# pasqal-io/Pulser

Measured on NVIDIA B200. Metric: time-steps/s (1 ns sampling intervals of the Sequence evolved per second), higher is better.
Workload: dtype f64 (complex128)

## Files before the change

pulser_b200/csrc/kernels.cuh:

```cuda
#pragma once
#include <cuda_runtime.h>
#include <stdint.h>

namespace pb200 {

struct c2 { double x, y; };

__host__ __device__ inline c2 cmul(c2 a, c2 b) { return {a.x * b.x - a.y * b.y, a.x * b.y + a.y * b.x}; }
__host__ __device__ inline c2 cadd(c2 a, c2 b) { return {a.x + b.x, a.y + b.y}; }

struct PassGeom {
    int n_bits;
    int lo_bits;
    int hi_shift;
    int hi_bits;
    uint32_t tile_flip_mask;
    unsigned long long extra_mask;
    int first_pass;
};

struct StageCoef {
    c2 c_psi, c_b2, c_g;
};

// ... 573 lines not shown
    for (unsigned long long em = g.extra_mask; em; em &= em - 1) {
        const int p = __ffsll((long long)em) - 1;
        const double sg = (((base >> p) & 1) == to_bit) ? 1.0 : -1.0;
        double2 raw[R];
#pragma unroll
        for (int r = 0; r < R; ++r) raw[r] = __ldg(reinterpret_cast<const double2*>(vsrc + (idx_of(r) ^ (1LL << p))));
#pragma unroll
        for (int r = 0; r < R; ++r) {
            pr[r] += raw[r].x; pi[r] += raw[r].y;
            if (!REAL_G) { qr[r] = fma(sg, raw[r].x, qr[r]); qi[r] = fma(sg, raw[r].y, qi[r]); }
        }
    }
    mbar_wait(&mbar, 0);
    const int jstart = __ffs(g.tile_flip_mask) - 1;
    c2 v[R];
#pragma unroll
    for (int r = 0; r < R; ++r) v[r] = tile[tid + r * NT];
    rb_tile_gather<true, REAL_G, TBITS, RB>(g, tile, nullptr, tid, to_bit, jstart, false, v, pr, pi, qr, qi);
#pragma unroll
    for (int r = 0; r < R; ++r) {
        double dx = a.u.g.x * pr[r], dy = a.u.g.x * pi[r];
        if (!REAL_G) { dx = fma(-a.u.g.y, qi[r], dx); dy = fma(a.u.g.y, qr[r], dy); }
        const c2 gv = {fma(dg[r], v[r].x, dx), fma(dg[r], v[r].y, dy)};
        const c2 res = cadd(part[r], cmul(a.coef.c_g, gv));
        st_c2(a.out + voff + idx_of(r), res);
        v[r] = res;
    }
    if (a.w_out) {
#pragma unroll
        for (int r = 0; r < R; ++r) {
            rtile[tid + r * NT] = v[r];
            pr[r] = 0.0; pi[r] = 0.0; qr[r] = 0.0; qi[r] = 0.0;
        }
        __syncthreads();
        rb_tile_gather<true, REAL_G, TBITS, RB>(g, rtile, nullptr, tid, to_bit, jstart, false, v, pr, pi, qr, qi);
#pragma unroll
        for (int r = 0; r < R; ++r) {
            const long long ix = idx_of(r);
            st_c2(a.w_out + voff + ix, c2{pr[r], pi[r]});
            if (!REAL_G) st_c2(a.w_out + a.w_plane + voff + ix, c2{qr[r], qi[r]});
        }
    }
}

#define PB200_TAYLOR_PMAX 8
struct TaylorArgs {
    const c2* v;
    c2* out;
    c2* g_out;
    c2* acc;
    const double* dint;
    long long dint_stride;
    long long D;
    PassGeom geo;
    c2 unit;
    const double* table;
    int to_bit, from_is_one;
    double th0, gam0, om0, m0;
    c2 scale;
    int nh;
    const c2* hchi[PB200_TAYLOR_PMAX];
    const c2* hg[PB200_TAYLOR_PMAX];
    double hth[PB200_TAYLOR_PMAX], hgam[PB200_TAYLOR_PMAX], hom[PB200_TAYLOR_PMAX], hm[PB200_TAYLOR_PMAX];
    int acc_read;
    int acc_add_v;
    int acc_on;
    c2 acc_mul;
};

template <int R>
__device__ __forceinline__ void taylor_epilogue(const TaylorArgs& a, const long long (&idx)[R], const c2 (&v)[R],
                                                const double (&gx)[R], const double (&gy)[R], const double (&off)[R],
                                                long long voff, const double* __restrict__ dsrc) {
    constexpr int H = (R >= 4) ? R / 2 : R;
    const int nb = a.geo.n_bits;
#pragma unroll
    for (int h0 = 0; h0 < R; h0 += H) {
        double sx[H], sy[H], cn[H];
        {
            double dv[H];
#pragma unroll
            for (int r = 0; r < H; ++r) dv[r] = dsrc ? __ldcs(dsrc + idx[h0 + r]) : 0.0;
#pragma unroll
            for (int r = 0; r < H; ++r) {
                const int ones = __popcll((unsigned long long)idx[h0 + r]);
                cn[r] = (double)(a.from_is_one ? ones : (nb - ones));
                const double diag = fma(-a.th0, cn[r], fma(-a.m0, off[h0 + r], dv[r] - a.gam0));
                sx[r] = fma(diag, v[h0 + r].x, a.om0 * gx[h0 + r]);
                sy[r] = fma(diag, v[h0 + r].y, a.om0 * gy[h0 + r]);
            }
        }
        for (int j = 0; j < a.nh; ++j) {
            if (a.hchi[j]) {
                c2 c[H];
#pragma unroll
                for (int r = 0; r < H; ++r) c[r] = ld_own(a.hchi[j] + voff + idx[h0 + r]);
#pragma unroll
                for (int r = 0; r < H; ++r) {
                    const double d = -fma(a.hth[j], cn[r], fma(a.hm[j], off[h0 + r], a.hgam[j]));
                    sx[r] = fma(d, c[r].x, sx[r]); sy[r] = fma(d, c[r].y, sy[r]);
                }
            }
            if (a.hg[j]) {
                c2 c[H];
#pragma unroll
                for (int r = 0; r < H; ++r) c[r] = ld_own(a.hg[j] + voff + idx[h0 + r]);
#pragma unroll
                for (int r = 0; r < H; ++r) { sx[r] = fma(a.hom[j], c[r].x, sx[r]); sy[r] = fma(a.hom[j], c[r].y, sy[r]); }
            }
        }
        c2 res[H];
#pragma unroll
        for (int r = 0; r < H; ++r) {
            res[r] = {a.scale.x * sx[r] - a.scale.y * sy[r], a.scale.x * sy[r] + a.scale.y * sx[r]};
            st_c2(a.out + voff + idx[h0 + r], res[r]);
            if (a.g_out) st_c2(a.g_out + voff + idx[h0 + r], c2{gx[h0 + r], gy[h0 + r]});
        }
        if (a.acc_on) {
            c2 ac[H];
#pragma unroll
            for (int r = 0; r < H; ++r) ac[r] = a.acc_read ? ld_own(a.acc + voff + idx[h0 + r]) : c2{0.0, 0.0};
#pragma unroll
            for (int r = 0; r < H; ++r) {
                c2 s = cadd(ac[r], res[r]);
                if (a.acc_add_v) s = cadd(s, v[h0 + r]);
                st_c2(a.acc + voff + idx[h0 + r], cmul(a.acc_mul, s));
            }
        }
    }
}

template <bool UNIFORM, bool REAL_G, int TBITS, int RB>
__global__ void __launch_bounds__(1 << (TBITS - RB), (65536 / ((1 << (TBITS - RB)) * (RB >= 3 ? 128 : 64))))
stage_d2_taylor_kernel(const __grid_constant__ TaylorArgs a) {
    constexpr int R = 1 << RB;
    constexpr int NT = 1 << (TBITS - RB);
    constexpr int TSIZE = 1 << TBITS;
    extern __shared__ __align__(128) unsigned char smem_raw[];
    c2* tile = reinterpret_cast<c2*>(smem_raw);
    __shared__ __align__(8) uint64_t mbar;
    const PassGeom& g = a.geo;
    const int tid = threadIdx.x;
    const long long traj = UNIFORM ? 0 : (long long)blockIdx.y;
    const long long voff = traj * a.D;
    const long long base = tile_base_of(g, blockIdx.x);
    const c2* vsrc = a.v + voff;

    if (tid == 0) mbar_init(&mbar, 1);
    __syncthreads();
    pdl_wait();
    pdl_launch_dependents();
    if (tid == 0) mbar_arrive_expect_tx(&mbar, (uint32_t)TSIZE * 16u);
    {
        const int rows = 1 << g.hi_bits;
        const uint32_t row_bytes = (uint32_t)(16u << g.lo_bits);
        for (int r = tid; r < rows; r += NT)
            tma_load_1d(tile + ((size_t)r << g.lo_bits), vsrc + base + ((long long)r << g.hi_shift), row_bytes, &mbar);
    }
    double* tab = reinterpret_cast<double*>(tile + TSIZE);
    if (!UNIFORM) {
        const int stride = d2_table_stride(g.n_bits);
        const double* src = a.table + traj * stride;
        for (int i = tid; i < stride; i += NT) tab[i] = src[i];
        __syncthreads();
    }
    const long long lomask = (1LL << g.lo_bits) - 1;
    const int to_bit = a.to_bit;
    c2 v[R];
    double pr[R], pi[R], qr[R], qi[R];
    long long idx[R];
#pragma unroll
    for (int r = 0; r < R; ++r) {
        const int t = tid + r * NT;
        idx[r] = base | (t & lomask) | ((long long)(t >> g.lo_bits) << g.hi_shift);
        pr[r] = 0.0; pi[r] = 0.0; qr[r] = 0.0; qi[r] = 0.0;
    }
    for (unsigned long long m = g.extra_mask; m; m &= m - 1) {
        const int p = __ffsll((long long)m) - 1;
        const int bit = (int)((base >> p) & 1);
        const double sg = (bit == to_bit) ? 1.0 : -1.0;
        double gx = 0.0, gy = 0.0;
        if (!UNIFORM) { gx = tab[2 * p]; gy = (bit == to_bit) ? tab[2 * p + 1] : -tab[2 * p + 1]; }
        double2 raw[R];
#pragma unroll
        for (int r = 0; r < R; ++r) raw[r] = __ldg(reinterpret_cast<const double2*>(vsrc + (idx[r] ^ (1LL << p))));
#pragma unroll
        for (int r = 0; r < R; ++r) {
            if (UNIFORM) {
                pr[r] += raw[r].x; pi[r] += raw[r].y;
                if (!REAL_G) { qr[r] = fma(sg, raw[r].x, qr[r]); qi[r] = fma(sg, raw[r].y, qi[r]); }
            } else {
                pr[r] = fma(gx, raw[r].x, pr[r]); pr[r] = fma(-gy, raw[r].y, pr[r]);
                pi[r] = fma(gx, raw[r].y, pi[r]); pi[r] = fma(gy, raw[r].x, pi[r]);
            }
        }
    }
    mbar_wait(&mbar, 0);
#pragma unroll
    for (int r = 0; r < R; ++r) v[r] = tile[tid + r * NT];
    rb_tile_gather<UNIFORM, REAL_G, TBITS, RB>(g, tile, tab, tid, to_bit, 0, false, v, pr, pi, qr, qi);
    double off[R];
    if (UNIFORM) {
#pragma unroll
        for (int r = 0; r < R; ++r) {
            const double dx = a.unit.x * pr[r], dy = a.unit.x * pi[r];
            if (!REAL_G) { pr[r] = fma(-a.unit.y, qi[r], dx); pi[r] = fma(a.unit.y, qr[r], dy); }
            else { pr[r] = dx; pi[r] = dy; }
            off[r] = 0.0;
        }
    } else {
        const int nb = g.n_bits;
        const long long fixed = base | (tid & lomask) | ((long long)(tid >> g.lo_bits) << g.hi_shift);
        double common = 0.0;
        for (int p = 0; p < nb; ++p) {
            const int bit = (int)((fixed >> p) & 1);
            common += (bit == a.from_is_one) ? tab[2 * nb + p] : 0.0;
        }
#pragma unroll
        for (int r = 0; r < R; ++r) {
            double acc = common;
#pragma unroll
            for (int q = 0; q < RB; ++q) {
                const int j = TBITS - RB + q;
                const int p = (j < g.lo_bits) ? j : (j - g.lo_bits + g.hi_shift);
                const double th = tab[2 * nb + p];
                const int bit = (r >> q) & 1;
                acc += ((bit == a.from_is_one) ? th : 0.0) - ((0 == a.from_is_one) ? th : 0.0);
            }
            off[r] = acc;
        }
    }
    taylor_epilogue<R>(a, idx, v, pr, pi, off, voff, a.dint ? a.dint + traj * a.dint_stride : nullptr);
}

__global__ void __launch_bounds__(256) stage_d2_taylor_small_kernel(const __grid_constant__ TaylorArgs a) {
    const long long s = (long long)blockIdx.x * blockDim.x + threadIdx.x;
    if (s >= a.D) return;
    const int nb = a.geo.n_bits;
    const long long traj = blockIdx.y;
    const long long voff = traj * a.D;
    const double* tab = a.table ? a.table + traj * d2_table_stride(nb) : nullptr;
    double gxs = 0.0, gys = 0.0, offv = 0.0;
    if (tab) {
        for (int p = 0; p < nb; ++p) {
            const double2 raw = __ldg(reinterpret_cast<const double2*>(a.v + voff + (s ^ (1LL << p))));
            const int bit = (int)((s >> p) & 1);
            const double gx = tab[2 * p], gy = (bit == a.to_bit) ? tab[2 * p + 1] : -tab[2 * p + 1];
            gxs = fma(gx, raw.x, gxs); gxs = fma(-gy, raw.y, gxs);
            gys = fma(gx, raw.y, gys); gys = fma(gy, raw.x, gys);
            offv += (bit == a.from_is_one) ? tab[2 * nb + p] : 0.0;
        }
    } else {
        double pr = 0.0, pi = 0.0, qr = 0.0, qi = 0.0;
        for (int p = 0; p < nb; ++p) {
            const double2 raw = __ldg(reinterpret_cast<const double2*>(a.v + voff + (s ^ (1LL << p))));
            const double sg = ((int)((s >> p) & 1) == a.to_bit) ? 1.0 : -1.0;
            pr += raw.x; pi += raw.y; qr = fma(sg, raw.x, qr); qi = fma(sg, raw.y, qi);
        }
        gxs = fma(-a.unit.y, qi, a.unit.x * pr);
        gys = fma(a.unit.y, qr, a.unit.x * pi);
    }
    const long long idx[1] = {s};
    const double2 own = __ldg(reinterpret_cast<const double2*>(a.v + voff + s));
    const c2 v[1] = {{own.x, own.y}};
    const double gx[1] = {gxs}, gy[1] = {gys}, off[1] = {offv};
    taylor_epilogue<1>(a, idx, v, gx, gy, off, voff, a.dint ? a.dint + traj * a.dint_stride : nullptr);
}

__host__ __device__ inline int gen_table_stride(int n, int n_drives) { return n_drives * 3 * n + 3; }

#define PB200_TILED_MAX_HIGH 40
#define PB200_MAX_DRIVES_K 3
struct GenArgs {
    const c2* v; const c2* psi; const c2* b2; c2* out;
    const double* dint; long long dint_stride; long long D;
    int n, dim, n_drives;
    int to[3], from[3];
    StageCoef coef;
    const double* table;
    const double* beta_dev;
    const double* xy; long long xy_stride; int xy_u, xy_d;
    unsigned long long slm_mask; const double* dint2;
    double* dot_acc;
    LanczosFuse lz;
};

__global__ void __launch_bounds__(256) stage_generic_kernel(GenArgs a) {
    extern __shared__ __align__(16) unsigned char smem_raw[];
    double* tab = reinterpret_cast<double*>(smem_raw);
    const int stride = gen_table_stride(a.n, a.n_drives);
    const long long traj = blockIdx.y;
    for (int i = threadIdx.x; i < stride; i += blockDim.x) tab[i] = a.table[traj * stride + i];
    __syncthreads();
    double* xys = tab + stride;
    if (a.xy) {
        const double wx = tab[stride - 2], wxc = tab[stride - 3];
        for (int i = threadIdx.x; i < a.n * a.n; i += blockDim.x) {
            const int qi = i / a.n, qj = i - qi * a.n;
            const bool touched = ((a.slm_mask >> qi) | (a.slm_mask >> qj)) & 1ULL;
            xys[i] = a.xy[traj * a.xy_stride + i] * (touched ? wxc : wx);
        }
        __syncthreads();
    }
    const double w = tab[stride - 2], gamma = tab[stride - 1];
    const long long voff = traj * a.D;
    for (long long idx = blockIdx.x * (long long)blockDim.x + threadIdx.x; idx < a.D;
         idx += (long long)gridDim.x * blockDim.x) {
        const c2 vo = a.v[voff + idx];
        double diag = -gamma;
        if (a.dint) diag = fma(w, a.dint[traj * a.dint_stride + idx], diag);
        if (a.dint2) diag = fma(tab[stride - 3], a.dint2[traj * a.dint_stride + idx], diag);
        double rr = 0.0, ri = 0.0;
        long long rem = idx, st = 1;
        for (int k = a.n - 1; k >= 0; --k) {
            const int digit = (int)(rem % a.dim);
            rem /= a.dim;
            for (int q = 0; q < a.n_drives; ++q) {
                const double* gq = tab + q * 3 * a.n;
                if (digit == a.to[q]) {
// ... 659 lines not shown
```

pulser_b200/csrc/plan.cu:

```cuda
#include <cuda_runtime.h>

#include <algorithm>
#include <map>
#include <mutex>
#include <unordered_map>
#include <cmath>
#include <complex>
#include <cstdarg>
#include <cstdio>
#include <cstdlib>
#include <cstring>
#include <stdexcept>
#include <string>
#include <vector>

#include "../../include/pulser_b200.h"
#include "kernels.cuh"
#include "spline.hpp"
#include <cub/device/device_scan.cuh>
#include <nvtx3/nvToolsExt.h>
#include <random>

namespace pb200 {

// ... 51 lines not shown
    std::multimap<size_t, void*> free_list[PB200_MAX_DEVICES];
    std::unordered_map<void*, size_t> size_of;
    size_t held[PB200_MAX_DEVICES] = {0};
};
static DevicePool& pool() { static DevicePool* p = new DevicePool(); return *p; }

static void* pool_alloc(int dev, size_t bytes) {
    if (bytes == 0) bytes = 16;
    bytes = (bytes + 255) & ~(size_t)255;
    DevicePool& pl = pool();
    if (dev >= 0 && dev < PB200_MAX_DEVICES) {
        std::lock_guard<std::mutex> lk(pl.mu);
        auto it = pl.free_list[dev].lower_bound(bytes);
        if (it != pl.free_list[dev].end() && it->first <= bytes + bytes / 4) {
            void* p = it->second;
            pl.held[dev] -= it->first;
            pl.free_list[dev].erase(it);
            return p;
        }
    }
    void* p = nullptr;
    cudaError_t e = cudaMalloc(&p, bytes);
    if (e != cudaSuccess) {
        cudaGetLastError();
        {
            std::lock_guard<std::mutex> lk(pl.mu);
            if (dev >= 0 && dev < PB200_MAX_DEVICES) {
                for (auto& kv : pl.free_list[dev]) { pl.size_of.erase(kv.second); cudaFree(kv.second); }
                pl.free_list[dev].clear(); pl.held[dev] = 0;
            }
        }
        CUDA_CHECK(cudaMalloc(&p, bytes));
    }
    std::lock_guard<std::mutex> lk(pl.mu);
    pl.size_of[p] = bytes;
    return p;
}

static void pool_free(int dev, void* p) {
    if (!p) return;
    DevicePool& pl = pool();
    static const size_t cap = (size_t)std::max(0, env_int("PB200_POOL_MIB", 16384)) << 20;
    {
        std::lock_guard<std::mutex> lk(pl.mu);
        auto it = pl.size_of.find(p);
        if (it != pl.size_of.end() && dev >= 0 && dev < PB200_MAX_DEVICES && pl.held[dev] + it->second <= cap) {
            pl.free_list[dev].emplace(it->second, p);
            pl.held[dev] += it->second;
            return;
        }
        if (it != pl.size_of.end()) pl.size_of.erase(it);
    }
    cudaFree(p);
}

static int device_setup(int dev) {
    static std::mutex mu;
    static int sm_count[PB200_MAX_DEVICES] = {0};
    std::lock_guard<std::mutex> lk(mu);
    if (dev >= 0 && dev < PB200_MAX_DEVICES && sm_count[dev] > 0) return sm_count[dev];
    int sms = 0;
    CUDA_CHECK(cudaDeviceGetAttribute(&sms, cudaDevAttrMultiProcessorCount, dev));
    const int max_smem = (1 << 13) * 16 + 1024;
    CUDA_CHECK(cudaFuncSetAttribute(stage_d2_kernel<true, true>, cudaFuncAttributeMaxDynamicSharedMemorySize, max_smem));
    CUDA_CHECK(cudaFuncSetAttribute(stage_d2_kernel<true, false>, cudaFuncAttributeMaxDynamicSharedMemorySize, max_smem));
    CUDA_CHECK(cudaFuncSetAttribute(stage_d2_kernel<false, false>, cudaFuncAttributeMaxDynamicSharedMemorySize, max_smem));
#define PB200_RB_ATTR(TB, RB)                                                                                                            \
    CUDA_CHECK(cudaFuncSetAttribute(stage_d2_rb_kernel<true, true, TB, RB>, cudaFuncAttributeMaxDynamicSharedMemorySize, max_smem));   \
    CUDA_CHECK(cudaFuncSetAttribute(stage_d2_rb_kernel<true, false, TB, RB>, cudaFuncAttributeMaxDynamicSharedMemorySize, max_smem));  \
    CUDA_CHECK(cudaFuncSetAttribute(stage_d2_rb_kernel<false, false, TB, RB>, cudaFuncAttributeMaxDynamicSharedMemorySize, max_smem));
    PB200_RB_ATTR(11, 2) PB200_RB_ATTR(11, 3) PB200_RB_ATTR(12, 2) PB200_RB_ATTR(12, 3)
#undef PB200_RB_ATTR
    CUDA_CHECK(cudaFuncSetAttribute(stage_d2_taylor_kernel<true, true, 11, 3>, cudaFuncAttributeMaxDynamicSharedMemorySize, 2048 * 16 + 256));
    CUDA_CHECK(cudaFuncSetAttribute(stage_d2_taylor_kernel<true, false, 11, 3>, cudaFuncAttributeMaxDynamicSharedMemorySize, 2048 * 16 + 256));
    CUDA_CHECK(cudaFuncSetAttribute(stage_d2_taylor_kernel<false, false, 11, 3>, cudaFuncAttributeMaxDynamicSharedMemorySize, 2048 * 16 + 2048));
    CUDA_CHECK(cudaFuncSetAttribute(stage_d2_fwd_kernel<true, 11, 3>, cudaFuncAttributeMaxDynamicSharedMemorySize, 2 * 2048 * 16 + 256));
    CUDA_CHECK(cudaFuncSetAttribute(stage_d2_fwd_kernel<false, 11, 3>, cudaFuncAttributeMaxDynamicSharedMemorySize, 2 * 2048 * 16 + 256));
    if (dev >= 0 && dev < PB200_MAX_DEVICES) sm_count[dev] = sms;
    return sms;
}

struct DriveTables {
    std::vector<PiecewiseCubic<cplx>> coef;
    std::vector<PiecewiseCubic<double>> det;
    std::vector<double> coef_scale, det_scale;
};

struct Plan {
    pb200_plan_desc desc;
    std::vector<double> times;
    int n = 0, dim = 0, B = 1;
    long long D = 0;
    int n_drives = 0;
    cudaStream_t stream = nullptr;
    bool own_stream = false;
    c2* buf[3] = {nullptr, nullptr, nullptr};
    c2* aux[6] = {nullptr, nullptr, nullptr, nullptr, nullptr, nullptr};
    int cur = 0;
    double* dint = nullptr;
    bool dint_shared = true;
    bool has_interaction = false;
    double* d_table = nullptr;
    size_t d_table_cap = 0;
    double* d_scratch = nullptr;
    std::vector<std::vector<DriveTables>> tabs;
    std::vector<std::vector<bool>> tabs_set;
    std::vector<double> dmin_cnt, dmax_cnt;
    std::vector<double> dmin_traj, dmax_traj;
    bool state_set = false;
    int tile_bits = 12;
    int max_extra = 3;
    int sm_count = 148;
    bool force_v1 = false;
    int reg_bits = 3;
    bool use_dual = true;
    std::vector<std::vector<cplx>> diss_gen;
    c2* kry = nullptr; int kry_cap = 0;
    double* d_kry = nullptr;
    int m_last = 8;
    bool use_krylov = false;
    long long kry_iters = 0;
    bool has_diss = false;
    std::vector<std::vector<cplx>> jump_ops;
    std::vector<std::vector<double>> jump_ldl;
    std::vector<std::vector<cplx>> jump_ldl_full;
    bool jump_diag = true;
    bool has_collapse = false;
    double* d_xy = nullptr; bool xy_shared = true; bool has_xy = false; int xy_u = 0, xy_d = 1;
// ... 1047 lines not shown
            for (int dgt = 0; P.jump_diag && dgt < P.dim; ++dgt) {
                CUDA_CHECK(cudaMemsetAsync(d_occ, 0, sizeof(double) * P.n, P.stream));
                const long long nb = std::min<long long>((P.D + 255) / 256, (long long)P.sm_count * 4);
                occupation_kernel<<<(unsigned)std::max<long long>(nb, 1), 256, sizeof(double) * P.n, P.stream>>>(
                    psi, d_occ, P.D, P.n, P.dim, dgt);
                CUDA_CHECK(cudaMemcpyAsync(occ.data() + (size_t)dgt * P.n, d_occ, sizeof(double) * P.n, cudaMemcpyDeviceToHost, P.stream));
            }
            CUDA_CHECK(cudaStreamSynchronize(P.stream));
            for (size_t op = 0; P.jump_diag && op < P.jump_ops.size(); ++op)
                for (int k = 0; k < P.n; ++k) {
                    double wv = 0.0;
                    for (int dgt = 0; dgt < P.dim; ++dgt) wv += P.jump_ldl[op][dgt] * occ[(size_t)dgt * P.n + k];
                    wts[op * P.n + k] = wv; tot += wv;
                }
            if (tot <= 0.0) { P.thresholds[tr] = uni(P.rng); continue; }
            double x = uni(P.rng) * tot; size_t sel = 0;
            for (; sel + 1 < wts.size(); ++sel) { x -= wts[sel]; if (x <= 0.0) break; }
            const size_t op = sel / P.n; const int k = (int)(sel % P.n);
            QuditOp qo{};
            for (int q = 0; q < P.dim * P.dim; ++q) qo.m[q] = {P.jump_ops[op][q].real(), P.jump_ops[op][q].imag()};
            long long stq = 1;
            for (int q = 0; q < P.n - 1 - k; ++q) stq *= P.dim;
            const double scale = 1.0 / std::sqrt(std::max(wts[sel], 1e-300));
            const long long nb = std::min<long long>((P.D / P.dim + 255) / 256, (long long)P.sm_count * 8);
            qudit_op_kernel<<<(unsigned)std::max<long long>(nb, 1), 256, 0, P.stream>>>(psi, P.D, P.dim, stq, scale, qo);
            CUDA_CHECK(cudaGetLastError());
            st.n_launches += 1 + P.dim;
            P.thresholds[tr] = uni(P.rng);
            P.jump_count[tr] += 1;
        }
        t = b;
    }
    norms2();
    for (int tr = 0; tr < P.B; ++tr) {
        if (norms[tr] <= 0.0) continue;
        const double sc = 1.0 / std::sqrt(norms[tr]);
        scale_kernel<<<(unsigned)std::max<long long>(blocks, 1), 256, 0, P.stream>>>(P.buf[P.cur] + (size_t)tr * P.D, P.D, sc);
        P.thresholds[tr] /= norms[tr];
        P.thresholds[tr] = std::min(P.thresholds[tr], 1.0);
    }
    CUDA_CHECK(cudaGetLastError());
    pool_free(P.desc.device, d_occ);
    CUDA_CHECK(cudaEventRecord(ev1, P.stream));
    CUDA_CHECK(cudaEventSynchronize(ev1));
    float ms = 0.f;
    CUDA_CHECK(cudaEventElapsedTime(&ms, ev0, ev1));
    st.gpu_ms = ms; st.integrator = 1; st.mean_step_samples = K;
    if (stats) *stats = st;
}

static thread_local const char* g_taylor_why = "";
static bool taylor_prepare(Plan& P);
static bool taylor_worthwhile(Plan& P, double gtol);
static bool taylor_geometry(const Plan& P, const std::vector<PassGeom>& passes, bool& use_rb);
static void propagate_taylor(Plan& P, double t_start, double t_stop, const pb200_run_opts* o, pb200_run_stats* stats);

static void propagate(Plan& P, double t_start, double t_stop, const pb200_run_opts* o, pb200_run_stats* stats) {
    if (!P.state_set) fail(PB200_ERR_STATE, "pb200_propagate: no state set (call pb200_state_set first)");
    for (int tr = 0; tr < P.B; ++tr)
        for (int q = 0; q < P.n_drives; ++q)
            if (!P.tabs_set[tr][q]) fail(PB200_ERR_STATE, "pb200_propagate: drive %d of trajectory %d not set", q, tr);
    const double tlo = P.times.front(), thi = P.times.back();
    const double eps = 1e-12;
    if (t_start < tlo - eps || t_stop > thi + eps || t_stop < t_start)
        fail(PB200_ERR_INVALID, "pb200_propagate: [%g, %g] outside sampling times [%g, %g]", t_start, t_stop, tlo, thi);
    t_start = std::max(t_start, tlo); t_stop = std::min(t_stop, thi);
    if (P.has_collapse) { propagate_mcwf(P, t_start, t_stop, o, stats); return; }
    {
        const int req = o ? o->integrator : 0;
        if (req < 0 || req > 3) fail(PB200_ERR_INVALID, "integrator must be 0 (auto), 1, 2 or 3");
        bool want = req == 3;
        if (req == 0 && P.use_taylor) {
            const bool steered = o && (o->max_step_samples > 0 || o->tol < 0.0 || o->extrapolate < 0 || o->check_every > 0 ||
                                       o->cheb_tol > 0.0 || (o->magnus_order != 0 && o->magnus_order != 4));
            want = !steered && t_stop > t_start;
        }
        if (want) {
            bool use_rb = false;
            const bool ok = taylor_prepare(P) && taylor_geometry(P, plan_passes(P.n, P.tile_bits, P.max_extra), use_rb) &&
                            (req == 3 || taylor_worthwhile(P, (o && o->tol > 0.0) ? o->tol : 1e-8));
            if (ok) { propagate_taylor(P, t_start, t_stop, o, stats); return; }
            if (env_int("PB200_TAYLOR_LOG", 0)) fprintf(stderr, "taylor not taken: %s\n", g_taylor_why);
            if (req == 3)
                fail(PB200_ERR_UNSUPPORTED, "integrator 3 (Taylor) needs a d = 2 register whose drive is one time shape of constant phase "
                                            "(per-qubit static factors / detuning offsets allowed), no collapse operators / SLM mask");
        }
    }
    const double gtol = (o && o->tol != 0.0) ? o->tol : (P.has_diss ? 1e-6 : 1e-8);
    const bool extrap = !(o && o->extrapolate < 0);
    const bool adaptive = gtol > 0.0;
    int Kmax = (o && o->max_step_samples > 0) ? o->max_step_samples
                                               : env_int("PB200_MAX_STEP", adaptive ? (extrap ? 32 : 16) : 4);
    int W = (o && o->refine_window >= 0) ? o->refine_window : env_int("PB200_REFINE_WINDOW", 8);
    const double tol_user = (o && o->cheb_tol > 0) ? o->cheb_tol : 0.0;
    double rtol = (o && o->rough_tol > 0) ? o->rough_tol : 1e-4;
    int order = (o && o->magnus_order) ? o->magnus_order : 4;
    int check_every = (o && o->check_every > 0) ? o->check_every : 12;
    if (order != 2 && order != 4) fail(PB200_ERR_INVALID, "magnus_order must be 2 or 4");

    pb200_run_stats st{};
    const std::vector<PassGeom> passes = plan_passes(P.n, P.tile_bits, P.max_extra);
    if (!P.fine_cache.valid || P.fine_cache.window != W || P.fine_cache.rtol != rtol) {
        P.fine_cache.fine = fine_intervals(P, W, rtol, 0.05, P.fine_cache.jump, P.fine_cache.dist);
        for (size_t i = 0; i < P.fine_cache.fine.size(); ++i) if (P.fine_cache.jump[i]) P.fine_cache.fine[i] = 1;
        P.fine_cache.window = W; P.fine_cache.rtol = rtol; P.fine_cache.valid = true;
    }
    const std::vector<char>& jump = P.fine_cache.jump;
    const std::vector<int>& dist = P.fine_cache.dist;
    const std::vector<char>& fine = P.fine_cache.fine;
    const double magnus_tol = 1e-11;
    const int nt = (int)P.times.size();
    const double rate_allowed = adaptive ? gtol / std::max(thi - tlo, 1e-30) : 0.0;
    auto cheb_tol_for = [&](double h, bool check) {
        if (tol_user > 0.0) return tol_user;
        if (!adaptive) return 1e-12;
        const double share = rate_allowed * h;
        return std::min(1e-12, std::max(2e-15, (check ? 0.01 : 0.2) * share));
    };

    EventPair evs;
    cudaEvent_t ev0 = evs.a, ev1 = evs.b;
    CUDA_CHECK(cudaEventRecord(ev0, P.stream));

    Program prog;
    auto flush = [&]() {
        if (prog.cheb.empty()) return;
        run_program(P, prog, passes, st);
        CUDA_CHECK(cudaStreamSynchronize(P.stream));
        prog = Program();
    };
    const size_t flush_doubles = (size_t)8 << 20;
    const size_t state_bytes = sizeof(c2) * (size_t)P.D * P.B;
// ... 469 lines not shown
    }
    std::vector<ld> mono(m, 0.0L), Tm2(m, 0.0L), Tm1(m, 0.0L), Tk(m, 0.0L);
    Tm2[0] = 1.0L;
    mono[0] += ck[0];
    if (m > 1) { Tm1[1] = 1.0L; for (int i = 0; i < m; ++i) mono[i] += ck[1] * Tm1[i]; }
    for (int k = 2; k < m; ++k) {
        for (int i = 0; i < m; ++i) Tk[i] = (i > 0 ? 2.0L * Tm1[i - 1] : 0.0L) - Tm2[i];
        for (int i = 0; i < m; ++i) mono[i] += ck[k] * Tk[i];
        Tm2 = Tm1; Tm1 = Tk;
    }
    std::vector<ld> cu(m, 0.0L), pw(m, 0.0L), nx(m, 0.0L);
    pw[0] = 1.0L;
    for (int k = 0; k < m; ++k) {
        for (int i = 0; i < m; ++i) cu[i] += mono[k] * pw[i];
        for (int i = 0; i < m; ++i) nx[i] = (i > 0 ? 2.0L * pw[i - 1] : 0.0L) - pw[i];
        pw = nx;
    }
    TaylorPoly out;
    out.c.resize(m);
    for (int i = 0; i < m; ++i) out.c[i] = (double)cu[i];
    const int ia = find_piece(x, a + 1e-15), ib = find_piece(x, a + h - 1e-15);
    const int npts = std::max(9, 4 * (ib - ia + 1) + 1);
    double r = 0.0;
    for (int q = 0; q < npts; ++q) {
        const double u = (double)q / (npts - 1);
        double pv = 0.0;
        for (int i = m - 1; i >= 0; --i) pv = pv * u + out.c[i];
        r = std::max(r, std::fabs(pv - eval_at(pc, x, a + h * u, order)));
    }
    out.resid = r;
    return out;
}

static int taylor_order(double h, const std::vector<double>& mj, double tol, double& tail_out) {
    const int p = (int)mj.size() - 1;
    std::vector<double> y(1, 1.0);
    const int kcap = 1200;
    for (int k = 0; k < kcap; ++k) {
        double s = 0.0;
        for (int j = 0; j <= std::min(p, k); ++j) s += mj[j] * y[k - j];
        y.push_back(h * s / (k + 1));
        if (k > 8 && y.back() < 1e-40 && y.back() < y[k]) break;
    }
    double tail = 0.0;
    int kk = (int)y.size() - 1;
    for (; kk >= 1; --kk) {
        if (tail + y[kk] > tol) break;
        tail += y[kk];
    }
    tail_out = tail;
    return std::max(kk, 1);
}

static void launch_taylor_stage(Plan& P, const PassGeom* geo, const TaylorArgs& a, long long& launches) {
    const bool uniform = a.table == nullptr;
    if (geo) {
        dim3 grid((unsigned)(P.D >> 11), (unsigned)(uniform ? 1 : P.B)), block(256);
        const size_t smem = (size_t)2048 * 16 + (uniform ? 0 : (size_t)d2_table_stride(P.n) * 8);
        const bool real_g = a.unit.y == 0.0;
        if (!uniform) launch_k(stage_d2_taylor_kernel<false, false, 11, 3>, grid, block, smem, P.stream, P.use_pdl, a);
        else if (real_g) launch_k(stage_d2_taylor_kernel<true, true, 11, 3>, grid, block, smem, P.stream, P.use_pdl, a);
        else launch_k(stage_d2_taylor_kernel<true, false, 11, 3>, grid, block, smem, P.stream, P.use_pdl, a);
    } else {
        dim3 grid((unsigned)((P.D + 255) / 256), (unsigned)P.B);
        stage_d2_taylor_small_kernel<<<grid, 256, 0, P.stream>>>(a);
    }
    ++launches;
}

static bool taylor_geometry(const Plan& P, const std::vector<PassGeom>& passes, bool& use_rb) {
    use_rb = passes.size() == 1 && passes[0].first_pass && passes[0].hi_bits == 0 && passes[0].lo_bits == 11 &&
             P.tile_bits == 11 && P.reg_bits == 3;
    return use_rb || P.n <= 16;
}

static void propagate_taylor(Plan& P, double t_start, double t_stop, const pb200_run_opts* o, pb200_run_stats* stats) {
    const double tlo = P.times.front(), thi = P.times.back();
    const double eps = 1e-12;
    const double gtol = (o && o->tol > 0.0) ? o->tol : 1e-8;
    const double rate = gtol / std::max(thi - tlo, 1e-30);
    const double rho_max = env_int("PB200_TAYLOR_RHO_MILLI", 14000) * 1e-3;
    const int pmax = std::min(PB200_TAYLOR_PMAX, std::max(1, env_int("PB200_TAYLOR_P", PB200_TAYLOR_PMAX)));
    const int order = P.desc.interp_order;
    const int N = P.n;
    const int nt = (int)P.times.size();
    const std::vector<PassGeom> passes = plan_passes(P.n, P.tile_bits, P.max_extra);
    bool use_rb = false;
    if (!taylor_geometry(P, passes, use_rb)) fail(PB200_ERR_UNSUPPORTED, "Taylor propagator: unsupported register size");
    const PiecewiseCubic<double>& om_pc = P.tay.om;
    const PiecewiseCubic<double>& th_pc = P.tabs[0][0].det[0];
    Plan::TaylorCache& C = P.tay;
    taylor_knot_widths(P);
    const double kRoundUnit = 0.05 * 1.1102230246251565e-16;
    double rho_target = rho_max;
    {
        double w_total = 0.0;
        for (int i = 0; i + 1 < nt; ++i) w_total += 0.5 * (C.w_knot[i] + C.w_knot[i + 1]) * (P.times[i + 1] - P.times[i]);
        for (int it = 0; it < 3; ++it) {
            const double n_est = std::max(w_total / std::max(rho_target, 1.0), 1.0);
            rho_target = std::min(rho_max, std::max(4.0, std::log(0.2 * gtol / (kRoundUnit * std::sqrt(n_est)))));
        }
    }
    double round2 = 0.0;
    const PiecewiseCubic<double>& m_pc = C.mshape;
    const double A_sum = std::max(C.a_sum_max, 1e-300), C_sum = std::max(C.c_sum_max, 1e-300);
    pb200_run_stats st{};
    EventPair evs;
    CUDA_CHECK(cudaEventRecord(evs.a, P.stream));
    ensure_aux_buffers(P);

    const double fit_total = 0.5 * rate * (t_stop - t_start);
    double fit_spent = 0.0;
    struct Fit { TaylorPoly om, th, m; bool ok; };
    auto fit_step = [&](double a, double h, bool single_piece) {
        Fit F; F.ok = false;
        const double budget = std::max(0.5 * rate * h, 0.02 * std::max(fit_total - fit_spent, 0.0));
        const double third = budget / (3.0 * h);
        auto one = [&](const PiecewiseCubic<double>& pc, TaylorPoly& out, double allow) {
            if (!single_piece) {
                out = taylor_fit(pc, P.times, order, a, h, pmax);
                if (out.resid > allow) return false;
            }
            for (int p = 0; p < pmax; ++p) {
                TaylorPoly f = taylor_fit(pc, P.times, order, a, h, p);
                if (f.resid <= allow || (single_piece && p >= 3)) { out = f; return true; }
            }
            if (single_piece) out = taylor_fit(pc, P.times, order, a, h, pmax);
            return true;
        };
        F.ok = one(om_pc, F.om, third / A_sum) && one(th_pc, F.th, third / N);
        if (F.ok && C.has_m) F.ok = one(m_pc, F.m, third / C_sum);
        if (!C.has_m) { F.m.c.assign(1, 0.0); F.m.resid = 0.0; }
        return F;
    };

    double t = t_start;
    double steps_len = 0.0;
    double t_retry_len = 0.0;
    const bool log_steps = env_int("PB200_TAYLOR_LOG", 0) != 0;
    while (t < t_stop - eps) {
        const int i0 = find_piece(P.times, t + eps);
// ... 52 lines not shown
        const int p = std::max(p_om, p_th);
        auto th_c = [&](int j) { return j < (int)F.th.c.size() ? F.th.c[j] : 0.0; };
        auto m_c = [&](int j) { return j < (int)F.m.c.size() ? F.m.c[j] : 0.0; };
        std::vector<double> gam(p + 1, 0.0), mj(p + 1, 0.0);
        {
            double c0, hw0;
            taylor_bounds(P, F.om.c[0], F.th.c[0], m_c(0), c0, hw0);
            gam[0] = c0; mj[0] = hw0;
            for (int j = 1; j <= p; ++j) {
                const double thj = th_c(j), omj = j <= p_om ? F.om.c[j] : 0.0;
                gam[j] = -thj * 0.5 * N;
                mj[j] = std::fabs(thj) * 0.5 * N + std::fabs(m_c(j)) * C_sum + std::fabs(omj) * A_sum;
            }
        }
        {
            double rho_eff = 0.0;
            for (int j = 0; j <= p; ++j) rho_eff += mj[j] / (j + 1);
            rho_eff *= h;
            if (rho_eff > 1.12 * rho_target && h > 1e-9) {
                t_retry_len = h * rho_target / rho_eff;
                continue;
            }
        }
        double trunc_bound = 0.0;
        const int K = taylor_order(h, mj, std::max(1e-15, 0.1 * rate * h), trunc_bound);
        const int n_chi = p_th + 2;
        const int n_g = p_om >= 1 ? p_om + 1 : 0;
        std::vector<c2**> free_slots;
        for (int i = 0; i < 3; ++i) if (i != P.cur) free_slots.push_back(&P.buf[i]);
        for (int i = 0; i < 6; ++i) free_slots.push_back(&P.aux[i]);
        const int need = (n_chi - 1) + n_g + 1;
        while ((int)free_slots.size() + (int)P.tay_ws.size() < need)
            P.tay_ws.push_back((c2*)pool_alloc(P.desc.device, sizeof(c2) * (size_t)P.D * P.B));
        for (size_t i = 0; i < P.tay_ws.size(); ++i) free_slots.push_back(&P.tay_ws[i]);
        std::vector<c2*> chi(n_chi), gr(n_g);
        int fs = 0;
        chi[0] = P.buf[P.cur];
        for (int i = 1; i < n_chi; ++i) chi[i] = *free_slots[fs++];
        for (int i = 0; i < n_g; ++i) gr[i] = *free_slots[fs++];
        c2** acc_slot = free_slots[fs++];
        c2* acc = *acc_slot;
        double phi = 0.0;
        for (int j = 0; j <= p; ++j) phi += gam[j] / (j + 1);
        phi *= h;
        long long launches = 0;
        for (int k = 0; k < K; ++k) {
            TaylorArgs a{};
            a.v = chi[k % n_chi]; a.out = chi[(k + 1) % n_chi];
            a.g_out = (n_g && k + 1 < K) ? gr[k % n_g] : nullptr;
            a.acc = acc;
            a.dint = P.has_interaction ? P.dint : nullptr;
            a.dint_stride = P.dint_shared ? 0 : P.D;
            a.D = P.D;
            a.geo = passes[0];
            a.unit = C.unit;
            a.table = C.uniform ? nullptr : C.d_tab;
            a.to_bit = P.desc.drives[0].state_to; a.from_is_one = P.desc.drives[0].state_from;
            a.th0 = F.th.c[0]; a.gam0 = gam[0]; a.om0 = F.om.c[0]; a.m0 = m_c(0);
            a.scale = {0.0, -h / (k + 1)};
            a.nh = std::min(p, k);
            for (int j = 1; j <= a.nh; ++j) {
                const double thj = th_c(j), mjv = m_c(j), omj = j <= p_om ? F.om.c[j] : 0.0;
                a.hth[j - 1] = thj; a.hgam[j - 1] = gam[j]; a.hom[j - 1] = omj; a.hm[j - 1] = mjv;
                a.hchi[j - 1] = (thj != 0.0 || mjv != 0.0 || gam[j] != 0.0) ? chi[(k - j) % n_chi] : nullptr;
                a.hg[j - 1] = (omj != 0.0) ? gr[(k - j) % n_g] : nullptr;
            }
            const bool last = (k + 1 == K);
            if ((k & 1) == 0) { a.acc_on = 1; a.acc_add_v = 1; a.acc_read = k > 0; }
            else { a.acc_on = last ? 1 : 0; a.acc_add_v = 0; a.acc_read = 1; }
            a.acc_mul = last ? c2{std::cos(phi), -std::sin(phi)} : c2{1.0, 0.0};
            launch_taylor_stage(P, use_rb ? &passes[0] : nullptr, a, launches);
        }
        CUDA_CHECK(cudaGetLastError());
        std::swap(P.buf[P.cur], *acc_slot);
        st.n_launches += launches; st.n_applies += K; st.n_exponentials += 1; ++st.n_steps;
        if (log_steps)
            fprintf(stderr, "taylor step t=%.6f h_ns=%.3f p_om=%d p_th=%d p_m=%d K=%d rho=%.3f resid=%.2e/%.2e/%.2e\n", t, h * 1e3, p_om,
                    p_th, p_m, K, mj[0] * h, F.om.resid, F.th.resid, F.m.resid);
        double rho_eff = 0.0;
        for (int j = 0; j <= p; ++j) rho_eff += mj[j] / (j + 1);
        st.max_rho = std::max(st.max_rho, rho_eff * h);
        const double fit_err = h * (A_sum * F.om.resid + N * F.th.resid + C_sum * F.m.resid);
        st.err_estimate += trunc_bound + fit_err;
        fit_spent += fit_err;
        { const double r = kRoundUnit * std::exp(std::min(rho_eff * h, 40.0)); round2 += r * r; }
        steps_len += h;
        t = b;
    }
    CUDA_CHECK(cudaEventRecord(evs.b, P.stream));
    CUDA_CHECK(cudaEventSynchronize(evs.b));
    float ms = 0.f;
    CUDA_CHECK(cudaEventElapsedTime(&ms, evs.a, evs.b));
    st.gpu_ms = ms;
    const double hi_mean = (thi - tlo) / std::max(nt - 1, 1);
    st.mean_step_samples = st.n_steps ? steps_len / st.n_steps / hi_mean : 0.0;
    st.err_estimate += std::sqrt(round2);
    st.integrator = 3;
    if (stats) *stats = st;
}

static ExpParams params_at(const Plan& P, double t) {
    ExpParams E;
    const int N = P.n, B = P.B, nd = P.n_drives;
    E.g.assign((size_t)B * nd * N, cplx(0)); E.th.assign((size_t)B * nd * N, 0.0); E.w = 1.0;
    if (P.has_slm) E.wc = eval_at(P.slm_coef, P.times, t, P.desc.interp_order);
    for (int tr = 0; tr < B; ++tr)
        for (int q = 0; q < nd; ++q) {
            const DriveTables& T = P.tabs[tr][q];
            const int rows = (int)T.coef.size();
            for (int k = 0; k < N; ++k) {
                const int r = rows == 1 ? 0 : k;
                E.g[pidx(P, tr, q, k)] = eval_at(T.coef[r], P.times, t, P.desc.interp_order);
                E.th[pidx(P, tr, q, k)] = eval_at(T.det[r], P.times, t, P.desc.interp_order);
            }
        }
    return E;
}

static void apply_h_device(Plan& P, double t, const c2* in, c2* out, long long& launches) {
    const bool d2path = is_d2path(P);
    const bool uniform = d2path && P.all_uniform() && P.B == 1;
    ExpParams E = params_at(P, t);
    std::vector<double> host;
    const int N = P.n;
// ... 786 lines not shown
```

Baseline: 36930.

## Make Taylor stage kernel persistent with double-buffered TMA tile prefetch

The Taylor stage kernel becomes a persistent grid-stride loop over (trajectory, tile) items. The next tile is prefetched with TMA into a second shared buffer while the current one is computed. Tile indexing assumes contiguous tiles (hi_bits==0), which simplifies index arithmetic, and non-uniform drives now use 4096-element tiles. The grid is capped at SM count (2x for uniform), which removes per-block launch and setup overhead. In exchange the kernel uses twice the shared memory, which limits occupancy, and adds a __syncthreads per item.

```diff
diff --git a/pulser_b200/csrc/kernels.cuh b/pulser_b200/csrc/kernels.cuh
--- a/pulser_b200/csrc/kernels.cuh
+++ b/pulser_b200/csrc/kernels.cuh
@@ -649,6 +649,7 @@
     const double* dint;
     long long dint_stride;
     long long D;
+    int n_traj;
     PassGeom geo;
     c2 unit;
     const double* table;
@@ -665,8 +666,8 @@
     c2 acc_mul;
 };
 
-template <int R>
-__device__ __forceinline__ void taylor_epilogue(const TaylorArgs& a, const long long (&idx)[R], const c2 (&v)[R],
+template <int R, int STEP>
+__device__ __forceinline__ void taylor_epilogue(const TaylorArgs& a, long long idx0, const c2 (&v)[R],
                                                 const double (&gx)[R], const double (&gy)[R], const double (&off)[R],
                                                 long long voff, const double* __restrict__ dsrc) {
     constexpr int H = (R >= 4) ? R / 2 : R;
@@ -677,10 +678,10 @@
         {
             double dv[H];
 #pragma unroll
-            for (int r = 0; r < H; ++r) dv[r] = dsrc ? __ldcs(dsrc + idx[h0 + r]) : 0.0;
+            for (int r = 0; r < H; ++r) dv[r] = dsrc ? __ldcs(dsrc + (idx0 + (h0 + r) * STEP)) : 0.0;
 #pragma unroll
             for (int r = 0; r < H; ++r) {
-                const int ones = __popcll((unsigned long long)idx[h0 + r]);
+                const int ones = __popcll((unsigned long long)(idx0 + (h0 + r) * STEP));
                 cn[r] = (double)(a.from_is_one ? ones : (nb - ones));
                 const double diag = fma(-a.th0, cn[r], fma(-a.m0, off[h0 + r], dv[r] - a.gam0));
                 sx[r] = fma(diag, v[h0 + r].x, a.om0 * gx[h0 + r]);
@@ -691,7 +692,7 @@
             if (a.hchi[j]) {
                 c2 c[H];
 #pragma unroll
-                for (int r = 0; r < H; ++r) c[r] = ld_own(a.hchi[j] + voff + idx[h0 + r]);
+                for (int r = 0; r < H; ++r) c[r] = ld_own(a.hchi[j] + voff + (idx0 + (h0 + r) * STEP));
 #pragma unroll
                 for (int r = 0; r < H; ++r) {
                     const double d = -fma(a.hth[j], cn[r], fma(a.hm[j], off[h0 + r], a.hgam[j]));
@@ -701,7 +702,7 @@
             if (a.hg[j]) {
                 c2 c[H];
 #pragma unroll
-                for (int r = 0; r < H; ++r) c[r] = ld_own(a.hg[j] + voff + idx[h0 + r]);
+                for (int r = 0; r < H; ++r) c[r] = ld_own(a.hg[j] + voff + (idx0 + (h0 + r) * STEP));
 #pragma unroll
                 for (int r = 0; r < H; ++r) { sx[r] = fma(a.hom[j], c[r].x, sx[r]); sy[r] = fma(a.hom[j], c[r].y, sy[r]); }
             }
@@ -710,77 +711,46 @@
 #pragma unroll
         for (int r = 0; r < H; ++r) {
             res[r] = {a.scale.x * sx[r] - a.scale.y * sy[r], a.scale.x * sy[r] + a.scale.y * sx[r]};
-            st_c2(a.out + voff + idx[h0 + r], res[r]);
-            if (a.g_out) st_c2(a.g_out + voff + idx[h0 + r], c2{gx[h0 + r], gy[h0 + r]});
+            st_c2(a.out + voff + (idx0 + (h0 + r) * STEP), res[r]);
+            if (a.g_out) st_c2(a.g_out + voff + (idx0 + (h0 + r) * STEP), c2{gx[h0 + r], gy[h0 + r]});
         }
         if (a.acc_on) {
             c2 ac[H];
 #pragma unroll
-            for (int r = 0; r < H; ++r) ac[r] = a.acc_read ? ld_own(a.acc + voff + idx[h0 + r]) : c2{0.0, 0.0};
+            for (int r = 0; r < H; ++r) ac[r] = a.acc_read ? ld_own(a.acc + voff + (idx0 + (h0 + r) * STEP)) : c2{0.0, 0.0};
 #pragma unroll
             for (int r = 0; r < H; ++r) {
                 c2 s = cadd(ac[r], res[r]);
                 if (a.acc_add_v) s = cadd(s, v[h0 + r]);
-                st_c2(a.acc + voff + idx[h0 + r], cmul(a.acc_mul, s));
+                st_c2(a.acc + voff + (idx0 + (h0 + r) * STEP), cmul(a.acc_mul, s));
             }
         }
     }
 }
 
 template <bool UNIFORM, bool REAL_G, int TBITS, int RB>
-__global__ void __launch_bounds__(1 << (TBITS - RB), (65536 / ((1 << (TBITS - RB)) * (RB >= 3 ? 128 : 64))))
-stage_d2_taylor_kernel(const __grid_constant__ TaylorArgs a) {
+__device__ __forceinline__ void taylor_tile(const TaylorArgs& a, const c2* tile, const double* __restrict__ tab,
+                                            long long base, long long traj, int tid, uint64_t* bar, uint32_t parity) {
     constexpr int R = 1 << RB;
     constexpr int NT = 1 << (TBITS - RB);
-    constexpr int TSIZE = 1 << TBITS;
-    extern __shared__ __align__(128) unsigned char smem_raw[];
-    c2* tile = reinterpret_cast<c2*>(smem_raw);
-    __shared__ __align__(8) uint64_t mbar;
     const PassGeom& g = a.geo;
-    const int tid = threadIdx.x;
-    const long long traj = UNIFORM ? 0 : (long long)blockIdx.y;
     const long long voff = traj * a.D;
-    const long long base = tile_base_of(g, blockIdx.x);
-    const c2* vsrc = a.v + voff;
-
-    if (tid == 0) mbar_init(&mbar, 1);
-    __syncthreads();
-    pdl_wait();
-    pdl_launch_dependents();
-    if (tid == 0) mbar_arrive_expect_tx(&mbar, (uint32_t)TSIZE * 16u);
-    {
-        const int rows = 1 << g.hi_bits;
-        const uint32_t row_bytes = (uint32_t)(16u << g.lo_bits);
-        for (int r = tid; r < rows; r += NT)
-            tma_load_1d(tile + ((size_t)r << g.lo_bits), vsrc + base + ((long long)r << g.hi_shift), row_bytes, &mbar);
-    }
-    double* tab = reinterpret_cast<double*>(tile + TSIZE);
-    if (!UNIFORM) {
-        const int stride = d2_table_stride(g.n_bits);
-        const double* src = a.table + traj * stride;
-        for (int i = tid; i < stride; i += NT) tab[i] = src[i];
-        __syncthreads();
-    }
-    const long long lomask = (1LL << g.lo_bits) - 1;
+    const long long s0 = base + tid;
     const int to_bit = a.to_bit;
     c2 v[R];
     double pr[R], pi[R], qr[R], qi[R];
-    long long idx[R];
-#pragma unroll
-    for (int r = 0; r < R; ++r) {
-        const int t = tid + r * NT;
-        idx[r] = base | (t & lomask) | ((long long)(t >> g.lo_bits) << g.hi_shift);
-        pr[r] = 0.0; pi[r] = 0.0; qr[r] = 0.0; qi[r] = 0.0;
-    }
+#pragma unroll
+    for (int r = 0; r < R; ++r) { pr[r] = 0.0; pi[r] = 0.0; qr[r] = 0.0; qi[r] = 0.0; }
     for (unsigned long long m = g.extra_mask; m; m &= m - 1) {
         const int p = __ffsll((long long)m) - 1;
         const int bit = (int)((base >> p) & 1);
         const double sg = (bit == to_bit) ? 1.0 : -1.0;
         double gx = 0.0, gy = 0.0;
         if (!UNIFORM) { gx = tab[2 * p]; gy = (bit == to_bit) ? tab[2 * p + 1] : -tab[2 * p + 1]; }
+        const c2* src = a.v + voff + (s0 ^ (1LL << p));
         double2 raw[R];
 #pragma unroll
-        for (int r = 0; r < R; ++r) raw[r] = __ldg(reinterpret_cast<const double2*>(vsrc + (idx[r] ^ (1LL << p))));
+        for (int r = 0; r < R; ++r) raw[r] = __ldg(reinterpret_cast<const double2*>(src + r * NT));
 #pragma unroll
         for (int r = 0; r < R; ++r) {
             if (UNIFORM) {
@@ -792,7 +762,7 @@
             }
         }
     }
-    mbar_wait(&mbar, 0);
+    mbar_wait(bar, parity);
 #pragma unroll
     for (int r = 0; r < R; ++r) v[r] = tile[tid + r * NT];
     rb_tile_gather<UNIFORM, REAL_G, TBITS, RB>(g, tile, tab, tid, to_bit, 0, false, v, pr, pi, qr, qi);
@@ -807,10 +777,9 @@
         }
     } else {
         const int nb = g.n_bits;
-        const long long fixed = base | (tid & lomask) | ((long long)(tid >> g.lo_bits) << g.hi_shift);
         double common = 0.0;
         for (int p = 0; p < nb; ++p) {
-            const int bit = (int)((fixed >> p) & 1);
+            const int bit = (int)((s0 >> p) & 1);
             common += (bit == a.from_is_one) ? tab[2 * nb + p] : 0.0;
         }
 #pragma unroll
@@ -818,16 +787,57 @@
             double acc = common;
 #pragma unroll
             for (int q = 0; q < RB; ++q) {
-                const int j = TBITS - RB + q;
-                const int p = (j < g.lo_bits) ? j : (j - g.lo_bits + g.hi_shift);
-                const double th = tab[2 * nb + p];
+                const double th = tab[2 * nb + TBITS - RB + q];
                 const int bit = (r >> q) & 1;
                 acc += ((bit == a.from_is_one) ? th : 0.0) - ((0 == a.from_is_one) ? th : 0.0);
             }
             off[r] = acc;
         }
     }
-    taylor_epilogue<R>(a, idx, v, pr, pi, off, voff, a.dint ? a.dint + traj * a.dint_stride : nullptr);
+    taylor_epilogue<R, NT>(a, s0, v, pr, pi, off, voff, a.dint ? a.dint + traj * a.dint_stride : nullptr);
+}
+
+template <bool UNIFORM, bool REAL_G, int TBITS, int RB>
+__global__ void __launch_bounds__(1 << (TBITS - RB), (65536 / ((1 << (TBITS - RB)) * 128)))
+stage_d2_taylor_kernel(const __grid_constant__ TaylorArgs a) {
+    constexpr int NT = 1 << (TBITS - RB);
+    constexpr int TSIZE = 1 << TBITS;
+    extern __shared__ __align__(128) unsigned char smem_raw[];
+    c2* tiles = reinterpret_cast<c2*>(smem_raw);
+    double* tabs = reinterpret_cast<double*>(tiles + 2 * TSIZE);
+    __shared__ __align__(8) uint64_t mbar[2];
+    const int tid = threadIdx.x;
+    const int stride = d2_table_stride(a.geo.n_bits);
+    const int tshift = a.geo.n_bits - TBITS;
+    const int n_items = a.n_traj << tshift;
+    auto fetch = [&](int item, int b) {
+        const long long traj = item >> tshift;
+        const long long base = (long long)(item & ((1 << tshift) - 1)) << TBITS;
+        if (tid == 0) {
+            mbar_arrive_expect_tx(&mbar[b], (uint32_t)TSIZE * 16u);
+            tma_load_1d(tiles + b * TSIZE, a.v + traj * a.D + base, (uint32_t)TSIZE * 16u, &mbar[b]);
+        }
+        if (!UNIFORM) {
+            const double* src = a.table + traj * stride;
+            for (int i = tid; i < stride; i += NT) tabs[b * stride + i] = src[i];
+        }
+    };
+
+    if (tid == 0) { mbar_init(&mbar[0], 1); mbar_init(&mbar[1], 1); }
+    __syncthreads();
+    pdl_wait();
+    pdl_launch_dependents();
+    int item = blockIdx.x;
+    fetch(item, 0);
+    if (!UNIFORM) __syncthreads();
+    for (int i = 0; item < n_items; ++i, item += gridDim.x) {
+        const int b = i & 1;
+        if (item + (int)gridDim.x < n_items) fetch(item + gridDim.x, b ^ 1);
+        taylor_tile<UNIFORM, REAL_G, TBITS, RB>(a, tiles + b * TSIZE, tabs + b * stride,
+                                                (long long)(item & ((1 << tshift) - 1)) << TBITS,
+                                                UNIFORM ? 0 : item >> tshift, tid, &mbar[b], (uint32_t)(i >> 1) & 1u);
+        __syncthreads();
+    }
 }
 
 __global__ void __launch_bounds__(256) stage_d2_taylor_small_kernel(const __grid_constant__ TaylorArgs a) {
@@ -857,11 +867,10 @@
         gxs = fma(-a.unit.y, qi, a.unit.x * pr);
         gys = fma(a.unit.y, qr, a.unit.x * pi);
     }
-    const long long idx[1] = {s};
     const double2 own = __ldg(reinterpret_cast<const double2*>(a.v + voff + s));
     const c2 v[1] = {{own.x, own.y}};
     const double gx[1] = {gxs}, gy[1] = {gys}, off[1] = {offv};
-    taylor_epilogue<1>(a, idx, v, gx, gy, off, voff, a.dint ? a.dint + traj * a.dint_stride : nullptr);
+    taylor_epilogue<1, 1>(a, s, v, gx, gy, off, voff, a.dint ? a.dint + traj * a.dint_stride : nullptr);
 }
 
 __host__ __device__ inline int gen_table_stride(int n, int n_drives) { return n_drives * 3 * n + 3; }
diff --git a/pulser_b200/csrc/plan.cu b/pulser_b200/csrc/plan.cu
--- a/pulser_b200/csrc/plan.cu
+++ b/pulser_b200/csrc/plan.cu
@@ -127,6 +127,11 @@
         if (it != pl.size_of.end()) pl.size_of.erase(it);
     }
     cudaFree(p);
+}
+
+static int taylor_tile_bits(bool uniform) { return uniform ? 11 : 12; }
+static size_t taylor_smem_bytes(int tbits, bool uniform, int n) {
+    return (size_t)2 * ((size_t)16 << tbits) + (uniform ? 0 : (size_t)2 * d2_table_stride(n) * sizeof(double));
 }
 
 static int device_setup(int dev) {
@@ -146,9 +151,9 @@
     CUDA_CHECK(cudaFuncSetAttribute(stage_d2_rb_kernel<false, false, TB, RB>, cudaFuncAttributeMaxDynamicSharedMemorySize, max_smem));
     PB200_RB_ATTR(11, 2) PB200_RB_ATTR(11, 3) PB200_RB_ATTR(12, 2) PB200_RB_ATTR(12, 3)
 #undef PB200_RB_ATTR
-    CUDA_CHECK(cudaFuncSetAttribute(stage_d2_taylor_kernel<true, true, 11, 3>, cudaFuncAttributeMaxDynamicSharedMemorySize, 2048 * 16 + 256));
-    CUDA_CHECK(cudaFuncSetAttribute(stage_d2_taylor_kernel<true, false, 11, 3>, cudaFuncAttributeMaxDynamicSharedMemorySize, 2048 * 16 + 256));
-    CUDA_CHECK(cudaFuncSetAttribute(stage_d2_taylor_kernel<false, false, 11, 3>, cudaFuncAttributeMaxDynamicSharedMemorySize, 2048 * 16 + 2048));
+    CUDA_CHECK(cudaFuncSetAttribute(stage_d2_taylor_kernel<true, true, 11, 3>, cudaFuncAttributeMaxDynamicSharedMemorySize, taylor_smem_bytes(11, true, 0)));
+    CUDA_CHECK(cudaFuncSetAttribute(stage_d2_taylor_kernel<true, false, 11, 3>, cudaFuncAttributeMaxDynamicSharedMemorySize, taylor_smem_bytes(11, true, 0)));
+    CUDA_CHECK(cudaFuncSetAttribute(stage_d2_taylor_kernel<false, false, 12, 3>, cudaFuncAttributeMaxDynamicSharedMemorySize, taylor_smem_bytes(12, false, PB200_MAX_QUDITS)));
     CUDA_CHECK(cudaFuncSetAttribute(stage_d2_fwd_kernel<true, 11, 3>, cudaFuncAttributeMaxDynamicSharedMemorySize, 2 * 2048 * 16 + 256));
     CUDA_CHECK(cudaFuncSetAttribute(stage_d2_fwd_kernel<false, 11, 3>, cudaFuncAttributeMaxDynamicSharedMemorySize, 2 * 2048 * 16 + 256));
     if (dev >= 0 && dev < PB200_MAX_DEVICES) sm_count[dev] = sms;
@@ -1302,7 +1307,7 @@
 static thread_local const char* g_taylor_why = "";
 static bool taylor_prepare(Plan& P);
 static bool taylor_worthwhile(Plan& P, double gtol);
-static bool taylor_geometry(const Plan& P, const std::vector<PassGeom>& passes, bool& use_rb);
+static bool taylor_geometry(const Plan& P, PassGeom& geo, bool& tiled);
 static void propagate_taylor(Plan& P, double t_start, double t_stop, const pb200_run_opts* o, pb200_run_stats* stats);
 
 static void propagate(Plan& P, double t_start, double t_stop, const pb200_run_opts* o, pb200_run_stats* stats) {
@@ -1326,8 +1331,9 @@
             want = !steered && t_stop > t_start;
         }
         if (want) {
-            bool use_rb = false;
-            const bool ok = taylor_prepare(P) && taylor_geometry(P, plan_passes(P.n, P.tile_bits, P.max_extra), use_rb) &&
+            PassGeom geo{};
+            bool tiled = false;
+            const bool ok = taylor_prepare(P) && taylor_geometry(P, geo, tiled) &&
                             (req == 3 || taylor_worthwhile(P, (o && o->tol > 0.0) ? o->tol : 1e-8));
             if (ok) { propagate_taylor(P, t_start, t_stop, o, stats); return; }
             if (env_int("PB200_TAYLOR_LOG", 0)) fprintf(stderr, "taylor not taken: %s\n", g_taylor_why);
@@ -1903,13 +1909,19 @@
     return std::max(kk, 1);
 }
 
-static void launch_taylor_stage(Plan& P, const PassGeom* geo, const TaylorArgs& a, long long& launches) {
+static void launch_taylor_stage(Plan& P, bool tiled, const TaylorArgs& a, long long& launches) {
     const bool uniform = a.table == nullptr;
-    if (geo) {
-        dim3 grid((unsigned)(P.D >> 11), (unsigned)(uniform ? 1 : P.B)), block(256);
-        const size_t smem = (size_t)2048 * 16 + (uniform ? 0 : (size_t)d2_table_stride(P.n) * 8);
+    if (tiled) {
+        const int tb = taylor_tile_bits(uniform);
+        const long long items = (P.D >> tb) * a.n_traj;
+#ifndef PB200_EXP_UNIFORM_ONE_ITEM
+        dim3 grid((unsigned)std::min<long long>(items, (long long)P.sm_count * (uniform ? 2 : 1))), block(1 << (tb - 3));
+#else
+        dim3 grid((unsigned)std::min<long long>(items, uniform ? items : P.sm_count)), block(1 << (tb - 3));
+#endif
+        const size_t smem = taylor_smem_bytes(tb, uniform, P.n);
         const bool real_g = a.unit.y == 0.0;
-        if (!uniform) launch_k(stage_d2_taylor_kernel<false, false, 11, 3>, grid, block, smem, P.stream, P.use_pdl, a);
+        if (!uniform) launch_k(stage_d2_taylor_kernel<false, false, 12, 3>, grid, block, smem, P.stream, P.use_pdl, a);
         else if (real_g) launch_k(stage_d2_taylor_kernel<true, true, 11, 3>, grid, block, smem, P.stream, P.use_pdl, a);
         else launch_k(stage_d2_taylor_kernel<true, false, 11, 3>, grid, block, smem, P.stream, P.use_pdl, a);
     } else {
@@ -1919,10 +1931,12 @@
     ++launches;
 }
 
-static bool taylor_geometry(const Plan& P, const std::vector<PassGeom>& passes, bool& use_rb) {
-    use_rb = passes.size() == 1 && passes[0].first_pass && passes[0].hi_bits == 0 && passes[0].lo_bits == 11 &&
-             P.tile_bits == 11 && P.reg_bits == 3;
-    return use_rb || P.n <= 16;
+static bool taylor_geometry(const Plan& P, PassGeom& geo, bool& tiled) {
+    const int tb = taylor_tile_bits(P.tay.uniform);
+    const std::vector<PassGeom> passes = plan_passes(P.n, tb, P.max_extra);
+    geo = passes[0];
+    tiled = P.n >= tb && passes.size() == 1 && geo.hi_bits == 0 && geo.lo_bits == tb;
+    return tiled || P.n <= 16;
 }
 
 static void propagate_taylor(Plan& P, double t_start, double t_stop, const pb200_run_opts* o, pb200_run_stats* stats) {
@@ -1935,9 +1949,9 @@
     const int order = P.desc.interp_order;
     const int N = P.n;
     const int nt = (int)P.times.size();
-    const std::vector<PassGeom> passes = plan_passes(P.n, P.tile_bits, P.max_extra);
-    bool use_rb = false;
-    if (!taylor_geometry(P, passes, use_rb)) fail(PB200_ERR_UNSUPPORTED, "Taylor propagator: unsupported register size");
+    PassGeom geo{};
+    bool tiled = false;
+    if (!taylor_geometry(P, geo, tiled)) fail(PB200_ERR_UNSUPPORTED, "Taylor propagator: unsupported register size");
     const PiecewiseCubic<double>& om_pc = P.tay.om;
     const PiecewiseCubic<double>& th_pc = P.tabs[0][0].det[0];
     Plan::TaylorCache& C = P.tay;
@@ -2096,7 +2110,8 @@
             a.dint = P.has_interaction ? P.dint : nullptr;
             a.dint_stride = P.dint_shared ? 0 : P.D;
             a.D = P.D;
-            a.geo = passes[0];
+            a.n_traj = C.uniform ? 1 : P.B;
+            a.geo = geo;
             a.unit = C.unit;
             a.table = C.uniform ? nullptr : C.d_tab;
             a.to_bit = P.desc.drives[0].state_to; a.from_is_one = P.desc.drives[0].state_from;
@@ -2113,7 +2128,7 @@
             if ((k & 1) == 0) { a.acc_on = 1; a.acc_add_v = 1; a.acc_read = k > 0; }
             else { a.acc_on = last ? 1 : 0; a.acc_add_v = 0; a.acc_read = 1; }
             a.acc_mul = last ? c2{std::cos(phi), -std::sin(phi)} : c2{1.0, 0.0};
-            launch_taylor_stage(P, use_rb ? &passes[0] : nullptr, a, launches);
+            launch_taylor_stage(P, tiled, a, launches);
         }
         CUDA_CHECK(cudaGetLastError());
         std::swap(P.buf[P.cur], *acc_slot);
```

Measured after the change: 36130 (median of 6 runs). -2.2%, worse.
